# pvachon/tsl-sdr

Measured on AMD Instinct MI355X. Metric: input IQ MSamp/s x channels demodulated, higher is better.
Workload: dtype int16

## Files before the change

tsl-sdr_amd/csrc/mfm_flex.hip:

```cpp
#include <hip/hip_runtime.h>

#include <cstdio>
#include <cstring>
#include <new>
#include <vector>

#include "../../include/multifm_hip.h"
#include "mfm_bch.h"

extern "C" __attribute__((visibility("hidden"))) void mfm_internal_set_error(const char *msg);

namespace {

constexpr uint32_t FX_HIST = 32768;
constexpr uint32_t FX_DEAD = 311;
constexpr uint32_t FX_MATCH_WORDS = 256;
constexpr uint32_t FX_HALO_WORDS = 10;
constexpr uint32_t FX_GATHER_THREADS = 256;

enum : uint32_t { FX_SEARCH = 0, FX_SYNC1 = 1, FX_FRAME = 2 };

struct FxCoding {
    uint16_t seq_a, baud;
    uint8_t levels, skip, fudge, nr_phases;
    uint16_t sync2, symbols;
};
__device__ const FxCoding fx_codings[4] = {
    { 0x78f3, 1600, 2, 9, 0, 1, 40, 2816 },
    { 0x84e7, 3200, 2, 4, 2, 2, 80, 5632 },
    { 0x4f97, 3200, 4, 9, 0, 2, 40, 2816 },
    { 0x215f, 6400, 4, 4, 2, 4, 80, 5632 },
};

struct FxIn {
    const int16_t *x;
    size_t stride;
    const int16_t *hist;
    uint64_t base, end;
};

__device__ __forceinline__ int fx_sample(const FxIn &I, uint32_t c, uint64_t s)
{
    const int16_t *in_block = I.x + (size_t)c * I.stride + (size_t)(s - I.base);
    const int16_t *in_ring = I.hist + (size_t)c * FX_HIST + (size_t)(s & (FX_HIST - 1));
    return *(s >= I.base ? in_block : in_ring);
}


struct __attribute__((packed, aligned(2))) FxPcm8 {
    int16_t v[8];
};

__device__ __forceinline__ uint32_t fx_sign8(const FxIn &I, uint32_t c, int64_t s)
{
    uint32_t b = 0;
    if (s >= (int64_t)I.base && (uint64_t)s + 8 <= I.end) {
        const FxPcm8 p = *reinterpret_cast<const FxPcm8 *>(I.x + (size_t)c * I.stride + (size_t)((uint64_t)s - I.base));
#pragma unroll
        for (int i = 0; i < 8; i++) {
            b |= (uint32_t)(p.v[i] >= 0) << i;
        }
    } else if (s >= 0 && (uint64_t)s + 8 <= I.base) {
        const uint4 q = *reinterpret_cast<const uint4 *>(I.hist + (size_t)c * FX_HIST + (size_t)((uint64_t)s & (FX_HIST - 1)));
        const uint32_t w[4] = { q.x, q.y, q.z, q.w };
#pragma unroll
        for (int i = 0; i < 4; i++) {
            b |= (uint32_t)((w[i] & 0x8000u) == 0) << (2 * i);
            b |= (uint32_t)((w[i] & 0x80000000u) == 0) << (2 * i + 1);
        }
    } else {
        for (int i = 0; i < 8; i++) {
            const int64_t si = s + i;
            if (si >= 0 && (uint64_t)si < I.end) {
                b |= (uint32_t)(fx_sample(I, c, (uint64_t)si) >= 0) << i;
            }
        }
    }
    return b;
}

__global__ __launch_bounds__(256) void fx_match_kernel(const FxIn I, uint32_t *M, uint32_t mstride, uint64_t *SUM, uint32_t sstride,
                                                       uint64_t w0, uint32_t nwords)
{
    __shared__ uint32_t bits[FX_MATCH_WORDS + FX_HALO_WORDS + 2];
    uint8_t *bytes = reinterpret_cast<uint8_t *>(bits);
    const uint32_t c = blockIdx.y, wb = blockIdx.x * FX_MATCH_WORDS, t = threadIdx.x;
    const int64_t s_first = ((int64_t)(w0 + wb) - (int64_t)FX_HALO_WORDS) * 32;
    for (uint32_t g = t; g < 4 * (FX_MATCH_WORDS + FX_HALO_WORDS); g += 256) {
        bytes[g] = (uint8_t)fx_sign8(I, c, s_first + 8 * (int64_t)g);
    }
    if (t == 0) {
        bits[FX_MATCH_WORDS + FX_HALO_WORDS] = 0;
    }
    __syncthreads();
    uint32_t m = 0;
    if (wb + t < nwords) {
        m = 0xffffffffu;
#pragma unroll
        for (uint32_t k = 0; k < 32; k++) {
            const uint32_t off = 32 * FX_HALO_WORDS + 32 * t - 10 * k;
            const uint32_t v = __funnelshift_r(bits[off >> 5], bits[(off >> 5) + 1], off & 31);
            m &= (k & 1) ? v : ~v;
        }
        const uint64_t i0 = (w0 + wb + t) * 32;
        if (i0 + 32 > I.end) {
            m &= (I.end > i0) ? (0xffffffffu >> (32 - (uint32_t)(I.end - i0))) : 0u;
        }
        M[(size_t)c * mstride + wb + t] = m;
    }
    const uint64_t any = __ballot(m != 0);
    if ((t & 63) == 0 && wb + t < nwords) {
        SUM[(size_t)c * sstride + ((wb + t) >> 6)] = any;
    }
}


struct FxState {
    uint64_t p;
    uint64_t j;
    uint32_t mode;
    uint32_t run;
    uint32_t eye;
    uint32_t coding;
    uint32_t a, b, inv_a, fiw_raw, fiw;
    int32_t range, delta;
    uint32_t cycle, frame, pad;
};

struct FxFrameDesc {
    uint64_t first;
    uint32_t coding;
    int32_t range, delta;
    uint32_t pad;
};

struct FxWalk {
    FxIn I;
    const uint32_t *M;
    const uint64_t *SUM;
    uint32_t mstride, sstride, nwords;
    uint64_t w0;
    FxState *st;
    mfm_flex_event *ev;
    mfm_flex_frame_words *fw;
    struct FxFrameDesc *fd;
    uint32_t *counts;
    uint32_t max_ev, max_fw;
    const MfmBchTables *bch;
};

__device__ __forceinline__ int fx_wave_sum(int v)
{
#pragma unroll
    for (int d = 32; d >= 1; d >>= 1) {
        v += __shfl_xor(v, d);
    }
    return v;
}

__device__ __forceinline__ uint32_t fx_checksum(uint32_t w)
{
    w &= 0x1fffffu;
    uint32_t s = 0;
#pragma unroll
    for (int n = 0; n < 6; n++) {
        s += (w >> (4 * n)) & 0xfu;
    }
    return s & 0xfu;
}

__device__ __forceinline__ uint32_t fx_slice4(int v, int delta, int range)
{
    const int s = (int16_t)(v - delta);
    if (s < 0) {
        return (-s > range / 4) ? 0u : 1u;
    }
    return (s > range / 4) ? 2u : 3u;
}

__device__ void fx_emit(const FxWalk &L, uint32_t c, uint32_t &nev, uint32_t type, uint64_t sample, const FxState &S, uint32_t fiw_rc,
                        uint32_t frame_index)
{
    if (nev < L.max_ev && threadIdx.x == 0) {
        mfm_flex_event e;
        e.type = type;
        e.channel = c;
        e.sample = sample;
        e.sync_sample = (type == MFM_FLEX_EV_FRAME) ? S.j : 0;
        e.coding = S.coding;
        e.baud = (S.coding < 4) ? fx_codings[S.coding].baud : 0;
        e.eye = S.eye;
        e.a = S.a;
        e.b = S.b;
        e.inv_a = S.inv_a;
        e.fiw_raw = S.fiw_raw;
        e.fiw = S.fiw;
        e.fiw_rc = fiw_rc;
        e.sample_range = S.range;
        e.sample_delta = S.delta;
        e.cycle = S.cycle;
        e.frame = S.frame;
        e.frame_index = frame_index;
        e.nr_phases = (S.coding < 4) ? fx_codings[S.coding].nr_phases : 0;
        e.reserved = 0;
        L.ev[(size_t)c * L.max_ev + nev] = e;
    }
    nev++;
}

__global__ __launch_bounds__(64) void fx_walk_kernel(const FxWalk L)
{
    const uint32_t c = blockIdx.x, lane = threadIdx.x;
    const FxIn &I = L.I;
    const uint64_t end = I.end;
    const uint32_t *M = L.M + (size_t)c * L.mstride;
    const uint64_t *SUM = L.SUM + (size_t)c * L.sstride;
    const uint32_t nsum = (L.nwords + 63) >> 6;
    __shared__ MfmBchTables bch_s;
    bool have_bch = false;
    FxState S = L.st[c];
    uint32_t nev = 0, nfw = 0;

    for (;;) {
        if (S.mode == FX_SEARCH) {
            bool opened = false;
            while (S.p < end) {
                if (S.run == 0) {
                    const uint32_t i = (uint32_t)((S.p >> 5) - L.w0);
                    const uint32_t head = M[i] & (0xffffffffu << (S.p & 31));
                    if (head != 0) {
                        S.p = (S.p & ~(uint64_t)31) + ((uint32_t)__ffs((int)head) - 1);
                    } else {
                        const uint32_t j = i + 1, sj = j >> 6;
                        uint64_t v = (sj + lane < nsum) ? SUM[sj + lane] : 0ull;
                        if (lane == 0) {
                            v &= ~0ull << (j & 63);
                        }
                        const uint64_t nz = __ballot(v != 0);
                        if (nz == 0) {
                            const uint64_t next = (L.w0 + (((uint64_t)sj + 64) << 6)) << 5;
                            S.p = next < end ? next : end;
                            continue;
                        }
                        const uint32_t fl = (uint32_t)__ffsll((unsigned long long)nz) - 1;
                        const uint32_t lo = (uint32_t)__shfl((int)(uint32_t)v, (int)fl), hi = (uint32_t)__shfl((int)(uint32_t)(v >> 32), (int)fl);
                        const uint64_t fv = (uint64_t)hi << 32 | lo;
                        const uint32_t wi = ((sj + fl) << 6) + ((uint32_t)__ffsll((unsigned long long)fv) - 1);
                        S.p = ((L.w0 + wi) << 5) + ((uint32_t)__ffs((int)M[wi]) - 1);
                    }
                }
                const uint32_t sh = (uint32_t)(S.p & 31);
                const uint32_t inv = ~(M[(S.p >> 5) - L.w0] >> sh);
                uint32_t avail = 32 - sh;
                if (end - S.p < avail) {
                    avail = (uint32_t)(end - S.p);
                }
                uint32_t ones = (uint32_t)__ffs((int)inv) - 1;
                if (inv == 0) {
                    ones = 32;
                }
                if (ones > avail) {
                    ones = avail;
                }
                S.run += ones;
                S.p += ones;
                if (ones < avail) {
                    const uint32_t cnt = S.run & 255u;
                    S.run = 0;
                    if (cnt >= 3) {
                        S.mode = FX_SYNC1;
                        S.j = S.p;
                        S.eye = cnt;
                        opened = true;
                        break;
                    }
                    S.p += 1;
                }
            }
            if (!opened) {
                break;
            }
        }

        if (S.mode == FX_SYNC1) {
            const uint64_t s0 = S.j + (10 - ((S.eye / 2) % 10));
            if (s0 + 790 >= end) {
                break;
            }
            const bool have_fiw = s0 + 1110 < end;
            const int v0 = fx_sample(I, c, s0 + 10 * lane);
            const uint32_t k1 = 64 + lane;
            const bool use1 = k1 < 80 || (have_fiw && k1 < 112);
            const int v1 = use1 ? fx_sample(I, c, s0 + 10 * k1) : 0;
            const uint64_t bal0 = __ballot(v0 >= 0), bal1 = __ballot(use1 && v1 >= 0);
            S.a = __brev((uint32_t)bal0);
// ... 9 lines not shown
            for (uint32_t i = 0; i < 4; i++) {
                if (S.coding == 0xffffffffu && __popc((uint32_t)fx_codings[i].seq_a ^ (S.a >> 16)) < 4) {
                    S.coding = i;
                }
            }
            if (S.coding == 0xffffffffu) {
                fx_emit(L, c, nev, MFM_FLEX_EV_BAD_BAUD, s0 + 790, S, 0, 0);
                S.mode = FX_SEARCH;
                S.run = 0;
                S.p = s0 + 790 + FX_DEAD;
                continue;
            }
            if (!have_fiw) {
                break;
            }
            S.fiw_raw = (uint32_t)(bal1 >> 16);
            const bool in1 = k1 < 112;
            const int sum_hi = fx_wave_sum((v0 > 0 ? v0 : 0) + (in1 && v1 > 0 ? v1 : 0));
            const int sum_lo = fx_wave_sum((v0 <= 0 ? v0 : 0) + (in1 && v1 <= 0 ? v1 : 0));
            const int n_hi = fx_wave_sum((v0 > 0) + (in1 && v1 > 0));
            const int n_lo = fx_wave_sum((v0 <= 0) + (in1 && v1 <= 0));
            const uint64_t f = s0 + 1110;
            uint32_t rc;
            if (n_hi == 0 || n_lo == 0) {
                rc = 3;
            } else {
                const int high = (int16_t)(sum_hi / n_hi), low = (int16_t)(sum_lo / n_lo);
                S.range = (int16_t)(high - low);
                S.delta = (int16_t)(high - S.range / 2);
                uint32_t bad;
                if (!have_bch) {
                    const uint32_t *src = reinterpret_cast<const uint32_t *>(L.bch);
                    uint32_t *dst = reinterpret_cast<uint32_t *>(&bch_s);
                    for (uint32_t i = lane; i < sizeof(MfmBchTables) / 4u; i += 64u) {
                        dst[i] = src[i];
                    }
                    have_bch = true;
                }
                S.fiw = mfm_bch_fix(&bch_s, S.fiw_raw & 0x7fffffffu, &bad);
                if (bad) {
                    rc = 1;
                } else if (fx_checksum(S.fiw) != 0xfu) {
                    rc = 2;
                } else {
                    rc = 0;
                    S.cycle = (S.fiw >> 4) & 0xfu;
                    S.frame = (S.fiw >> 8) & 0x7fu;
                }
            }
            if (rc != 0) {
                fx_emit(L, c, nev, MFM_FLEX_EV_BAD_FIW, f, S, rc, 0);
                S.mode = FX_SEARCH;
                S.run = 0;
                S.p = f + FX_DEAD;
                continue;
            }
            S.mode = FX_FRAME;
            S.j = f;
        }

        if (S.mode == FX_FRAME) {
            const FxCoding cd = fx_codings[S.coding];
            const uint32_t step = cd.skip + 1u;
            const uint64_t first = S.j + step + cd.fudge + (uint64_t)cd.sync2 * step;
            const uint64_t e = first + (uint64_t)(cd.symbols - 1u) * step;
            if (e >= end) {
                break;
            }
            if (nfw < L.max_fw && nev < L.max_ev && lane == 0) {
                L.fd[(size_t)c * L.max_fw + nfw] = FxFrameDesc{ first, S.coding, S.range, S.delta, 0u };
            }
            fx_emit(L, c, nev, MFM_FLEX_EV_FRAME, e, S, 0, nfw);
            nfw++;
            S.mode = FX_SEARCH;
            S.run = 0;
            S.p = e + FX_DEAD;
        }
    }

    if (lane == 0) {
        L.st[c] = S;
        L.counts[2 * c] = nev;
        L.counts[2 * c + 1] = nfw;
    }
}

__global__ __launch_bounds__(FX_GATHER_THREADS) void fx_gather_kernel(const FxWalk L)
{
    __shared__ uint8_t sym[5632];
    const uint32_t c = blockIdx.y, f = blockIdx.x;
    const uint32_t nfw = L.counts[2 * c + 1] < L.max_fw ? L.counts[2 * c + 1] : L.max_fw;
    if (f >= nfw) {
        return;
    }
    const FxFrameDesc d = L.fd[(size_t)c * L.max_fw + f];
    const FxCoding cd = fx_codings[d.coding];
    const uint32_t step = cd.skip + 1u;
    const bool four = cd.levels == 4;
    uint32_t *out = &L.fw[(size_t)c * L.max_fw + f].words[0][0];
#pragma unroll 11
    for (uint32_t k = threadIdx.x; k < cd.symbols; k += FX_GATHER_THREADS) {
        const int v = fx_sample(L.I, c, d.first + (uint64_t)k * step);
        sym[k] = (uint8_t)(four ? fx_slice4(v, d.delta, d.range) : (uint32_t)(v >= 0));
    }
    __syncthreads();
    for (uint32_t item = threadIdx.x; item < 4 * MFM_FLEX_PHASE_WORDS; item += FX_GATHER_THREADS) {
        const uint32_t q = item / MFM_FLEX_PHASE_WORDS, w = item % MFM_FLEX_PHASE_WORDS;
        bool present;
        uint32_t mul = 1, add = 0, sel = 0;
        if (cd.nr_phases == 1) {
            present = q == 0;
        } else if (cd.nr_phases == 2) {
            present = q == 0 || q == 2;
            if (four) {
                sel = q == 0;
            } else {
                mul = 2;
                add = q >> 1;
            }
        } else {
            present = true;
            mul = 2;
            add = q >> 1;
            sel = (q & 1) == 0;
        }
        uint32_t word = 0;
        if (present) {
            const uint32_t n0 = (w >> 3) * 256 + (w & 7);
#pragma unroll
            for (uint32_t jb = 0; jb < 32; jb++) {
                word |= (((uint32_t)sym[(n0 + 8 * jb) * mul + add] >> sel) & 1u) << jb;
            }
        }
        out[item] = word;
    }
}

__global__ __launch_bounds__(256) void fx_hist_kernel(int16_t *hist, const int16_t *x, size_t stride, uint64_t base, uint32_t n)
{
    const uint32_t c = blockIdx.y, k = blockIdx.x * 256 + threadIdx.x;
    const uint32_t cnt = n < FX_HIST ? n : FX_HIST;
    if (k < cnt) {
        const uint32_t off = n - cnt + k;
        hist[(size_t)c * FX_HIST + (size_t)((base + off) & (FX_HIST - 1))] = x[(size_t)c * stride + off];
    }
}

thread_local char g_fx_error[256] = "";

}

#define FX_TRY(expr)                                                                                         \
    do {                                                                                                     \
        hipError_t err_ = (expr);                                                                            \
        if (err_ != hipSuccess) {                                                                            \
            snprintf(g_fx_error, sizeof(g_fx_error), "%s failed: %s", #expr, hipGetErrorString(err_));       \
            mfm_internal_set_error(g_fx_error);                                                              \
            return MFM_E_DEVICE;                                                                             \
        }                                                                                                    \
    } while (0)

struct mfm_flex {
    mfm_flex_config cfg{};
    uint32_t max_ev = 0, max_fw = 0, mstride = 0, sstride = 0;
    int16_t *d_hist = nullptr;
    uint32_t *d_m = nullptr;
    uint64_t *d_sum = nullptr;
    FxState *d_st = nullptr;
    mfm_flex_event *d_ev = nullptr;
    mfm_flex_frame_words *d_fw = nullptr;
    FxFrameDesc *d_fd = nullptr;
    uint32_t *d_counts = nullptr;
    MfmBchTables *d_bch = nullptr;
    uint64_t total = 0;
    hipStream_t last_stream = nullptr;
    bool have_call = false;
};

extern "C" {

#define FX_TRY_C(expr)                                                                                       \
    do {                                                                                                     \
        hipError_t err_c_ = (expr);                                                                          \
        if (err_c_ != hipSuccess) {                                                                          \
            char msg_c_[256];                                                                                \
            snprintf(msg_c_, sizeof(msg_c_), "%s failed: %s", #expr, hipGetErrorString(err_c_));             \
            mfm_internal_set_error(msg_c_);                                                                  \
            mfm_flex_destroy(pf);                                                                            \
            return MFM_E_DEVICE;                                                                             \
        }                                                                                                    \
    } while (0)

int mfm_flex_create(struct mfm_flex **pf, const struct mfm_flex_config *cfg)
{
    if (!pf || !cfg) {
        return MFM_E_INVAL;
    }
    *pf = nullptr;
    if (cfg->abi_version != MFM_ABI_VERSION || 0 == cfg->nr_channels || 0 == cfg->max_in_samples ||
        cfg->max_in_samples > (1u << 26) || cfg->flags != 0) {
        return MFM_E_INVAL;
    }
    MfmBchTables *d_bch = nullptr;
    const int rc = mfm_internal_bch_device_tables(cfg->device, &d_bch);
    if (rc != MFM_OK) {
        return rc;
    }
    mfm_flex *f = new (std::nothrow) mfm_flex();
    if (!f) {
        return MFM_E_NOMEM;
    }
    f->cfg = *cfg;
    f->d_bch = d_bch;
    f->max_ev = cfg->max_events ? cfg->max_events : cfg->max_in_samples / 1024 + 8;
    f->max_fw = cfg->max_in_samples / 28672 + 2;
    if (f->max_fw > f->max_ev) {
        f->max_fw = f->max_ev;
    }
    f->mstride = cfg->max_in_samples / 32 + 4;
    f->sstride = f->mstride / 64 + 2;
    const size_t C = cfg->nr_channels;
    *pf = f;
    FX_TRY_C(hipSetDevice(cfg->device));
    FX_TRY_C(hipMalloc(&f->d_hist, C * FX_HIST * sizeof(int16_t)));
    FX_TRY_C(hipMemset(f->d_hist, 0, C * FX_HIST * sizeof(int16_t)));
    FX_TRY_C(hipMalloc(&f->d_m, C * f->mstride * sizeof(uint32_t)));
    FX_TRY_C(hipMalloc(&f->d_sum, C * f->sstride * sizeof(uint64_t)));
    FX_TRY_C(hipMalloc(&f->d_st, C * sizeof(FxState)));
    {
        std::vector<FxState> st(C);
        memset(st.data(), 0, C * sizeof(FxState));
        for (size_t c = 0; c < C; c++) {
            st[c].mode = FX_SEARCH;
            st[c].p = FX_DEAD - 1;
        }
        FX_TRY_C(hipMemcpy(f->d_st, st.data(), C * sizeof(FxState), hipMemcpyHostToDevice));
    }
    FX_TRY_C(hipMalloc(&f->d_ev, C * f->max_ev * sizeof(mfm_flex_event)));
    FX_TRY_C(hipMalloc(&f->d_fw, C * f->max_fw * sizeof(mfm_flex_frame_words)));
    FX_TRY_C(hipMalloc(&f->d_fd, C * f->max_fw * sizeof(FxFrameDesc)));
    FX_TRY_C(hipMalloc(&f->d_counts, C * 2 * sizeof(uint32_t)));
    FX_TRY_C(hipMemset(f->d_counts, 0, C * 2 * sizeof(uint32_t)));
    FX_TRY_C(hipDeviceSynchronize());
    return MFM_OK;
}

void mfm_flex_destroy(struct mfm_flex **pf)
{
    if (!pf || !*pf) {
        return;
    }
    mfm_flex *f = *pf;
    (void)hipSetDevice(f->cfg.device);
    (void)hipDeviceSynchronize();
    (void)hipFree(f->d_hist);
    (void)hipFree(f->d_m);
    (void)hipFree(f->d_sum);
    (void)hipFree(f->d_st);
    (void)hipFree(f->d_ev);
    (void)hipFree(f->d_fw);
    (void)hipFree(f->d_fd);
    (void)hipFree(f->d_counts);
    delete f;
    *pf = nullptr;
}

int mfm_flex_process_device(struct mfm_flex *f, const int16_t *d_pcm, size_t in_stride, size_t nr_in, void *stream)
{
    if (!f || (!d_pcm && nr_in) || nr_in > f->cfg.max_in_samples || (nr_in && in_stride < nr_in)) {
        return MFM_E_INVAL;
    }
    hipStream_t s = static_cast<hipStream_t>(stream);
    const uint32_t C = f->cfg.nr_channels, n = (uint32_t)nr_in;
    FX_TRY(hipSetDevice(f->cfg.device));
    if (f->have_call && f->last_stream != s) {
        FX_TRY(hipStreamSynchronize(f->last_stream));
    }
    f->last_stream = s;
    f->have_call = true;
    if (0 == n) {
        FX_TRY(hipMemsetAsync(f->d_counts, 0, (size_t)C * 2 * sizeof(uint32_t), s));
        return MFM_OK;
    }
    const FxIn in{ d_pcm, in_stride, f->d_hist, f->total, f->total + n };
    const uint64_t w0 = in.base >> 5;
    const uint32_t nwords = (uint32_t)(((in.end - 1) >> 5) - w0 + 1);
    hipLaunchKernelGGL(fx_match_kernel, dim3((nwords + FX_MATCH_WORDS - 1) / FX_MATCH_WORDS, C), dim3(256), 0, s, in, f->d_m,
                       f->mstride, f->d_sum, f->sstride, w0, nwords);
    FX_TRY(hipGetLastError());
    const FxWalk W{ in, f->d_m, f->d_sum, f->mstride, f->sstride, nwords, w0, f->d_st, f->d_ev, f->d_fw, f->d_fd, f->d_counts, f->max_ev, f->max_fw, f->d_bch };
    hipLaunchKernelGGL(fx_walk_kernel, dim3(C), dim3(64), 0, s, W);
    FX_TRY(hipGetLastError());
    const uint32_t fw_now = n / 28672u + 2u < f->max_fw ? n / 28672u + 2u : f->max_fw;
    hipLaunchKernelGGL(fx_gather_kernel, dim3(fw_now, C), dim3(FX_GATHER_THREADS), 0, s, W);
    FX_TRY(hipGetLastError());
    const uint32_t cnt = n < FX_HIST ? n : FX_HIST;
    hipLaunchKernelGGL(fx_hist_kernel, dim3((cnt + 255) / 256, C), dim3(256), 0, s, f->d_hist, d_pcm, in_stride, in.base, n);
    FX_TRY(hipGetLastError());
    f->total += n;
    return MFM_OK;
}

int mfm_flex_process_host(struct mfm_flex *f, const int16_t *pcm, size_t in_stride, size_t nr_in)
{
    if (!f || (!pcm && nr_in)) {
        return MFM_E_INVAL;
    }
    FX_TRY(hipSetDevice(f->cfg.device));
    const uint32_t C = f->cfg.nr_channels;
    int16_t *d_in = nullptr;
    FX_TRY(hipMalloc(&d_in, (size_t)C * (nr_in ? nr_in : 1) * 2));
    if (nr_in) {
        FX_TRY(hipMemcpy2D(d_in, nr_in * 2, pcm, in_stride * 2, nr_in * 2, C, hipMemcpyHostToDevice));
    }
    const int rc = mfm_flex_process_device(f, d_in, nr_in, nr_in, nullptr);
    (void)hipDeviceSynchronize();
    (void)hipFree(d_in);
    return rc;
}

int mfm_flex_seek(struct mfm_flex *f, uint64_t samples_before)
{
    if (!f) {
        mfm_internal_set_error("mfm_flex_seek: no object");
        return MFM_E_INVAL;
    }
    if (samples_before >= (1ull << 62)) {
        mfm_internal_set_error("mfm_flex_seek: samples_before must stay below 2^62 (the walk forms int64 differences of positions)");
        return MFM_E_INVAL;
    }
    FX_TRY(hipSetDevice(f->cfg.device));
    if (f->have_call) {
        FX_TRY(hipStreamSynchronize(f->last_stream));
    }
    const size_t C = f->cfg.nr_channels;
    std::vector<FxState> st(C);
    memset(st.data(), 0, C * sizeof(FxState));
    for (size_t c = 0; c < C; c++) {
        st[c].mode = FX_SEARCH;
        st[c].p = samples_before + (FX_DEAD - 1);
    }
    FX_TRY(hipMemset(f->d_hist, 0, C * FX_HIST * sizeof(int16_t)));
    FX_TRY(hipMemcpy(f->d_st, st.data(), C * sizeof(FxState), hipMemcpyHostToDevice));
    FX_TRY(hipMemset(f->d_counts, 0, C * 2 * sizeof(uint32_t)));
    FX_TRY(hipDeviceSynchronize());
    f->total = samples_before;
    f->last_stream = nullptr;
    f->have_call = false;
    return MFM_OK;
}

int mfm_flex_fetch_events(struct mfm_flex *f, struct mfm_flex_event *events, size_t max_events, size_t *nr_events,
                          struct mfm_flex_frame_words *frames, size_t max_frames, size_t *nr_frames)
{
    if (!f || !nr_events || !nr_frames || (!events && max_events) || (!frames && max_frames)) {
        return MFM_E_INVAL;
    }
    *nr_events = 0;
    *nr_frames = 0;
    if (!f->have_call) {
        return MFM_OK;
    }
    FX_TRY(hipSetDevice(f->cfg.device));
    FX_TRY(hipStreamSynchronize(f->last_stream));
    const uint32_t C = f->cfg.nr_channels;
    std::vector<uint32_t> cnt((size_t)C * 2);
    FX_TRY(hipMemcpy(cnt.data(), f->d_counts, (size_t)C * 2 * sizeof(uint32_t), hipMemcpyDeviceToHost));
    size_t tot_ev = 0, tot_fw = 0;
    bool overflow = false;
    for (uint32_t c = 0; c < C; c++) {
        overflow |= cnt[2 * c] > f->max_ev || cnt[2 * c + 1] > f->max_fw;
        tot_ev += cnt[2 * c] > f->max_ev ? f->max_ev : cnt[2 * c];
        tot_fw += cnt[2 * c + 1] > f->max_fw ? f->max_fw : cnt[2 * c + 1];
    }
    *nr_events = tot_ev;
    *nr_frames = tot_fw;
    if (tot_ev > max_events || tot_fw > max_frames) {
        return MFM_E_NOMEM;
    }
    size_t pe = 0, pw = 0;
    for (uint32_t c = 0; c < C; c++) {
        const uint32_t ke = cnt[2 * c] > f->max_ev ? f->max_ev : cnt[2 * c];
        const uint32_t kw = cnt[2 * c + 1] > f->max_fw ? f->max_fw : cnt[2 * c + 1];
        if (ke) {
            FX_TRY(hipMemcpy(events + pe, f->d_ev + (size_t)c * f->max_ev, (size_t)ke * sizeof(mfm_flex_event),
                             hipMemcpyDeviceToHost));
        }
        if (kw) {
            FX_TRY(hipMemcpy(frames + pw, f->d_fw + (size_t)c * f->max_fw, (size_t)kw * sizeof(mfm_flex_frame_words),
                             hipMemcpyDeviceToHost));
        }
        for (uint32_t i = 0; i < ke; i++) {
            mfm_flex_event *e = &events[pe + i];
            if (e->type == MFM_FLEX_EV_FRAME) {
                if (e->frame_index < kw) {
                    e->frame_index += (uint32_t)pw;
                } else {
                    overflow = true;
                    e->frame_index = 0xffffffffu;
                }
            }
        }
        pe += ke;
        pw += kw;
    }
    if (overflow) {
        snprintf(g_fx_error, sizeof(g_fx_error), "a channel produced more than max_events=%u events in one call", f->max_ev);
        mfm_internal_set_error(g_fx_error);
        return MFM_E_STATE;
    }
    return MFM_OK;
}

}
```

tsl-sdr_amd/csrc/mfm_resampler.hip:

```cpp
#include <hip/hip_runtime.h>

#include <cstdio>
#include <cstring>
#include <new>
#include <vector>

#include "../../include/multifm_hip.h"

extern "C" __attribute__((visibility("hidden"))) void mfm_internal_set_error(const char *msg);
#include "mfm_numerics.h"
#include "mfm_rs_plan.h"

namespace {

struct RsLaunch {
    const int16_t *tail;
    const int16_t *pcm;
    int16_t *y;
    const int16_t *phase;
    int16_t *tail_out;
    size_t in_stride;
    uint32_t tail_len, nr_in, tail_cap, out_cap, n_out, plen, interp, decim, p0, nchan, invert;
    uint32_t pos_end, new_tail;
    uint32_t *bits;
    uint32_t bits_stride;
};

template <int BITS>
__device__ __forceinline__ bool rs_pred(int32_t y)
{
    const int16_t s = (int16_t)y;
    return BITS == (int)MFM_BITS_NEG ? s < 0 : s > 0;
}

__device__ __forceinline__ int16_t rs_sample(const RsLaunch &L, uint32_t c, uint32_t v)
{
    int16_t s = 0;
    if (v < L.tail_len) {
        s = L.tail[(size_t)c * L.tail_cap + v];
    } else if (v - L.tail_len < L.nr_in) {
        s = L.pcm[(size_t)c * L.in_stride + (v - L.tail_len)];
    }
    return L.invert ? (int16_t)(-s) : s;
}

template <int NP, int BITS>
__global__ __launch_bounds__(RS_NT) void mfm_resample_kernel(const RsLaunch L)
{
    extern __shared__ __attribute__((aligned(16))) uint8_t rs_smem[];
    uint32_t *ph_s = reinterpret_cast<uint32_t *>(rs_smem);
    const uint32_t npairs = L.plen / 2u;
    int16_t *x_s = reinterpret_cast<int16_t *>(rs_smem + (size_t)L.interp * L.plen * 2u);
    const uint32_t c = blockIdx.y, tid = threadIdx.x;
    const uint32_t j0 = blockIdx.x * RS_OPB;
    const uint32_t j1 = (j0 + RS_OPB < L.n_out ? j0 + RS_OPB : L.n_out) - 1u;
    const uint32_t in_lo = ((L.p0 + j0 * L.decim) / L.interp) & ~1u;
    const uint32_t in_hi = (L.p0 + j1 * L.decim) / L.interp + L.plen + 2u + 8u;
    for (uint32_t i = tid; i < L.interp * npairs; i += RS_NT) {
        ph_s[i] = reinterpret_cast<const uint32_t *>(L.phase)[i];
    }
    for (uint32_t v = in_lo + tid; v < in_hi; v += RS_NT) {
        x_s[v - in_lo] = rs_sample(L, c, v);
    }
    __syncthreads();
    const uint32_t *x32 = reinterpret_cast<const uint32_t *>(x_s);

    const uint32_t t_first = L.p0 + (j0 + tid) * L.decim;
    uint32_t pos_abs = t_first / L.interp, ph = t_first - pos_abs * L.interp;
    const uint32_t step_pos = (RS_NT * L.decim) / L.interp, step_ph = (RS_NT * L.decim) % L.interp;
    constexpr bool REGCOEF = NP > 0;
    uint32_t cw[REGCOEF ? NP : 1];
    if (REGCOEF) {
#pragma unroll
        for (uint32_t i = 0; i < (uint32_t)NP; i++) {
            cw[i] = i < npairs ? ph_s[ph * npairs + i] : 0u;
        }
    }
#pragma unroll
    for (uint32_t u = 0; u < RS_OPT; u++) {
        const uint32_t j = j0 + tid + u * RS_NT;
        if (j >= L.n_out) {
            break;
        }
        const uint32_t pos = pos_abs - in_lo;
        const uint32_t *xw = x32 + (pos >> 1);
        const uint32_t sh = (pos & 1u) * 16u;
        int32_t acc = 0;
        uint32_t lo = xw[0];
        if (REGCOEF) {
#pragma unroll
            for (uint32_t i = 0; i < (uint32_t)NP; i++) {
                const uint32_t hi = xw[i + 1];
                const uint32_t pr = __builtin_amdgcn_alignbit(hi, lo, sh);
                asm("v_dot2_i32_i16 %0, %1, %2, %0" : "+v"(acc) : "v"(pr), "v"(cw[i]));
                lo = hi;
            }
        } else {
            const uint32_t *cp = ph_s + ph * npairs;
            for (uint32_t i = 0; i < npairs; i++) {
                const uint32_t hi = xw[i + 1];
                const uint32_t pr = __builtin_amdgcn_alignbit(hi, lo, sh);
                asm("v_dot2_i32_i16 %0, %1, %2, %0" : "+v"(acc) : "v"(pr), "v"(cp[i]));
                lo = hi;
            }
        }
        asm volatile("s_nop 2" : "+v"(acc));
        if (BITS) {
            const unsigned long long m = __ballot(rs_pred<BITS>(mfm_r14_wide(acc)));
            if ((tid & 31u) == 0) {
                L.bits[(size_t)c * L.bits_stride + (j >> 5)] = (uint32_t)(m >> (tid & 32u));
            }
        } else {
            L.y[(size_t)c * L.out_cap + j] = (int16_t)mfm_r14_wide(acc);
        }
        pos_abs += step_pos;
        ph += step_ph;
        if (ph >= L.interp) {
            ph -= L.interp;
            pos_abs += 1u;
        }
    }
}

__global__ void mfm_rs_tail_kernel(const RsLaunch L)
{
    const uint32_t c = blockIdx.x;
    for (uint32_t i = threadIdx.x; i < L.new_tail; i += blockDim.x) {
        int16_t s = 0;
        const uint32_t v = L.pos_end + i;
        if (v < L.tail_len) {
            s = L.tail[(size_t)c * L.tail_cap + v];
        } else if (v - L.tail_len < L.nr_in) {
            s = L.pcm[(size_t)c * L.in_stride + (v - L.tail_len)];
        }
        L.tail_out[(size_t)c * L.tail_cap + i] = s;
    }
}


typedef int rs_v4i __attribute__((ext_vector_type(4)));

struct RsMLaunch {
    RsLaunch b;
    const rs_v4i *gfrag;
    const int32_t *krow;
    uint32_t R;
    uint32_t rp;
    uint32_t plane;
};

struct __attribute__((packed, aligned(2))) RsPcm8 {
    int16_t v[8];
};

template <int KS, int BITS>
__global__ __launch_bounds__(RSM_NT) void mfm_resample_mfma_kernel(const RsMLaunch M)
{
    extern __shared__ __attribute__((aligned(16))) uint8_t rs_smem[];
    const RsLaunch &L = M.b;
    uint8_t *const pl_h = rs_smem, *const pl_l = rs_smem + M.plane;
    const uint32_t c = blockIdx.y, tid = threadIdx.x, lane = tid & 63u, wave = tid >> 6;
    const uint32_t b0 = blockIdx.x * RSM_NB;
    const uint32_t nrows = RSM_NB + (64u * KS + M.rp - 1u) / M.rp;
    const uint32_t v0 = b0 * M.R;

    const uint32_t g8 = (M.R + 7u) / 8u;
    for (uint32_t it = tid; it < nrows * g8; it += RSM_NT) {
        const uint32_t row = it / g8, grp = it - row * g8;
        const uint32_t v = v0 + row * M.R + 8u * grp;
        uint32_t w[4];
        if (v >= L.tail_len && v + 8u <= L.tail_len + L.nr_in) {
            const RsPcm8 p = *reinterpret_cast<const RsPcm8 *>(L.pcm + (size_t)c * L.in_stride + (v - L.tail_len));
#pragma unroll
            for (int i = 0; i < 4; i++) {
                w[i] = mfm_pack16(p.v[2 * i], p.v[2 * i + 1]);
            }
            if (L.invert) {
#pragma unroll
                for (int i = 0; i < 4; i++) {
                    w[i] = mfm_pack16(-(int32_t)p.v[2 * i], -(int32_t)p.v[2 * i + 1]);
                }
            }
        } else {
#pragma unroll
            for (int i = 0; i < 4; i++) {
                w[i] = mfm_pack16(rs_sample(L, c, v + 2u * (uint32_t)i), rs_sample(L, c, v + 2u * (uint32_t)i + 1u));
            }
        }
        uint2 lo, hi;
        lo.x = __builtin_amdgcn_perm(w[1], w[0], 0x06040200u) ^ 0x80808080u;
        lo.y = __builtin_amdgcn_perm(w[3], w[2], 0x06040200u) ^ 0x80808080u;
        hi.x = __builtin_amdgcn_perm(w[1], w[0], 0x07050301u);
        hi.y = __builtin_amdgcn_perm(w[3], w[2], 0x07050301u);
        const uint32_t at = row * M.rp + 8u * grp;
        *reinterpret_cast<uint2 *>(pl_l + at) = lo;
        *reinterpret_cast<uint2 *>(pl_h + at) = hi;
    }
    __syncthreads();

    const uint32_t kg = lane >> 4, n = lane & 15u;
    rs_v4i a_h[KS], a_l[KS];
#pragma unroll
    for (int ks = 0; ks < KS; ks++) {
        a_h[ks] = M.gfrag[(0 * KS + ks) * 64 + lane];
        a_l[ks] = M.gfrag[(1 * KS + ks) * 64 + lane];
    }
    rs_v4i kr;
#pragma unroll
    for (int i = 0; i < 4; i++) {
        kr[i] = M.krow[4u * kg + (uint32_t)i];
    }
    uint32_t nibw[4] = { 0, 0, 0, 0 };
#pragma unroll
    for (uint32_t g = 0; g < 4; g++) {
        const uint32_t blk = wave * 64u + g * 16u + n;
        const uint32_t off = blk * M.rp + 16u * kg;
        rs_v4i hh = { 0, 0, 0, 0 }, md = hh, ll = hh;
#pragma unroll
        for (int ks = 0; ks < KS; ks++) {
            const rs_v4i b_h = *reinterpret_cast<const rs_v4i *>(pl_h + off + 64u * ks);
            const rs_v4i b_l = *reinterpret_cast<const rs_v4i *>(pl_l + off + 64u * ks);
            hh = __builtin_amdgcn_mfma_i32_16x16x64_i8(a_h[ks], b_h, hh, 0, 0, 0);
            md = __builtin_amdgcn_mfma_i32_16x16x64_i8(a_h[ks], b_l, md, 0, 0, 0);
            ll = __builtin_amdgcn_mfma_i32_16x16x64_i8(a_l[ks], b_l, ll, 0, 0, 0);
            md = __builtin_amdgcn_mfma_i32_16x16x64_i8(a_l[ks], b_h, md, 0, 0, 0);
        }
        const uint32_t j = 16u * (b0 + blk) + 4u * kg;
        int32_t y[4];
#pragma unroll
        for (int i = 0; i < 4; i++) {
            const uint32_t acc = (uint32_t)ll[i] + ((uint32_t)md[i] << 8) + ((uint32_t)hh[i] << 16) + (uint32_t)kr[i];
            y[i] = mfm_r14_wide((int32_t)acc);
        }
        if (BITS) {
            uint32_t nib = 0;
#pragma unroll
            for (int i = 0; i < 4; i++) {
                nib |= (rs_pred<BITS>(y[i]) && j + (uint32_t)i < L.n_out ? 1u : 0u) << i;
            }
            nibw[g] = nib << (16u * (n & 1u) + 4u * kg);
            continue;
        }
        int16_t *dst = L.y + (size_t)c * L.out_cap + j;
        if (j + 4u <= L.n_out) {
            uint2 w;
            w.x = mfm_pack16(y[0], y[1]);
            w.y = mfm_pack16(y[2], y[3]);
            *reinterpret_cast<uint2 *>(dst) = w;
        } else {
#pragma unroll
            for (int i = 0; i < 4; i++) {
                if (j + (uint32_t)i < L.n_out) {
                    dst[i] = (int16_t)y[i];
                }
            }
        }
    }
    if (BITS) {
        const bool b5 = (lane & 32u) != 0u, b4 = (lane & 16u) != 0u;
        uint32_t k0 = b5 ? nibw[2] : nibw[0], k1 = b5 ? nibw[3] : nibw[1];
        k0 |= (uint32_t)__shfl_xor((int)(b5 ? nibw[0] : nibw[2]), 32);
        k1 |= (uint32_t)__shfl_xor((int)(b5 ? nibw[1] : nibw[3]), 32);
        uint32_t k = b4 ? k1 : k0;
        k |= (uint32_t)__shfl_xor((int)(b4 ? k0 : k1), 16);
        k |= (uint32_t)__shfl_xor((int)k, 1);
        const uint32_t wi = (b0 >> 1) + 32u * wave + 8u * kg + (n >> 1);
        if ((n & 1u) == 0u && 32u * wi < L.n_out) {
            L.bits[(size_t)c * L.bits_stride + wi] = k;
        }
    }
}

struct DcState {
    int32_t x_n_1, y_n_1, acc;
};

__global__ __launch_bounds__(64) void mfm_dc_block_kernel(int16_t *y, uint32_t out_cap, uint32_t n_out, uint32_t nchan, int32_t p,
                                                          DcState *st)
{
    const uint32_t c = blockIdx.x * blockDim.x + threadIdx.x;
    if (c >= nchan) {
        return;
    }
    const DcState s0 = st[c];
    uint32_t r = (uint32_t)s0.acc - (uint32_t)s0.x_n_1;
    int32_t yp = s0.y_n_1, xl = 0;
    int16_t *yy = y + (size_t)c * out_cap;
    uint32_t i = 0;
    constexpr uint32_t V = 8;
    if (n_out >= 8u * V) {
        typedef uint32_t u32x4 __attribute__((ext_vector_type(4)));
        const u32x4 *src = reinterpret_cast<const u32x4 *>(yy);
        u32x4 *dst = reinterpret_cast<u32x4 *>(yy);
        u32x4 cur[V], nxt[V];
#pragma unroll
        for (uint32_t k = 0; k < V; k++) {
            cur[k] = src[k];
        }
        const int32_t np = -p;
        for (; i + 8u * V <= n_out; i += 8u * V) {
            const u32x4 *pn = src + (i + 16u * V <= n_out ? i / 8u + V : i / 8u);
#pragma unroll
            for (uint32_t k = 0; k < V; k++) {
                nxt[k] = pn[k];
            }
#pragma unroll
            for (uint32_t k = 0; k < V; k++) {
                const u32x4 w = cur[k];
                u32x4 o;
#pragma unroll
                for (int d = 0; d < 4; d++) {
                    uint32_t acc;
                    r += (uint32_t)__mul24(yp, np);
                    asm("v_mad_i32_i16 %0, %1, %2, %3 op_sel:[0,0,0,0]" : "=v"(acc) : "v"(w[d]), "s"(16384), "v"(r));
                    yp = (int32_t)acc >> 14;
                    const uint32_t lo = (uint32_t)yp;
                    r += (uint32_t)__mul24(yp, np);
                    asm("v_mad_i32_i16 %0, %1, %2, %3 op_sel:[1,0,0,0]" : "=v"(acc) : "v"(w[d]), "s"(16384), "v"(r));
                    yp = (int32_t)acc >> 14;
                    o[d] = __builtin_amdgcn_perm((uint32_t)yp, lo, 0x05040100u);
                }
                xl = (int32_t)w[3] >> 16;
                dst[i / 8u + k] = o;
            }
#pragma unroll
            for (uint32_t k = 0; k < V; k++) {
                cur[k] = nxt[k];
            }
        }
    }
    for (; i < n_out; i++) {
        r -= (uint32_t)p * (uint32_t)yp;
        xl = (int32_t)yy[i];
        yp = (int32_t)(((uint32_t)xl << 14) + r) >> 14;
        yy[i] = (int16_t)yp;
    }
    if (n_out) {
        DcState s;
        s.x_n_1 = (int32_t)((uint32_t)xl << 14);
        s.acc = (int32_t)(((uint32_t)xl << 14) + r);
        s.y_n_1 = yp;
        st[c] = s;
    }
}

thread_local char g_rs_error[256] = "";

}

struct mfm_resampler {
    mfm_resampler_config cfg{};
    RsPlan plan;
// ... 172 lines not shown
        const uint32_t row = kk / p.rp, col = kk % p.rp;
        if (col < p.R) {
            const size_t v = (size_t)row * p.R + col;
            const int32_t s = v < nr_x ? x[v] : 0;
            pl_l[kk] = (int8_t)((s & 0xff) ^ 0x80);
            pl_h[kk] = (int8_t)(s >> 8);
        }
    }
    const int8_t *a_h = t.frag.data() + ((size_t)phase * 2u + 0u) * p.ks * 64u * 16u;
    const int8_t *a_l = t.frag.data() + ((size_t)phase * 2u + 1u) * p.ks * 64u * 16u;
    for (uint32_t q = 0; q < 16; q++) {
        uint32_t hh = 0, md = 0, ll = 0;
        for (uint32_t ks = 0; ks < p.ks; ks++) {
            for (uint32_t kgq = 0; kgq < 4; kgq++) {
                const size_t fa = ((size_t)ks * 64u + kgq * 16u + q) * 16u;
                const uint32_t off = 16u * kgq + 64u * ks;
                for (uint32_t j = 0; j < 16; j++) {
                    const int32_t ah = a_h[fa + j], al = a_l[fa + j], bh = pl_h[off + j], bl = pl_l[off + j];
                    hh += (uint32_t)(ah * bh);
                    md += (uint32_t)(ah * bl) + (uint32_t)(al * bh);
                    ll += (uint32_t)(al * bl);
                }
            }
        }
        const uint32_t acc = ll + (md << 8) + (hh << 16) + (uint32_t)t.krow[(size_t)phase * 16u + q];
        y16[q] = (int16_t)mfm_r14_wide((int32_t)acc);
    }
    return MFM_OK;
}

}

template <int BITS>
static int rs_process(mfm_resampler *r, const int16_t *d_pcm, size_t in_stride, size_t nr_in, hipStream_t s, uint32_t *pn_out)
{
    const uint32_t C = r->cfg.nr_channels, I = r->cfg.interpolate, D = r->cfg.decimate;
    const uint32_t total = r->tail + (uint32_t)nr_in;
    uint32_t n_out = 0;
    if (total > r->plen) {
        const uint64_t lim = (uint64_t)(total - r->plen) * I;
        if (lim > r->phase_id) {
            n_out = (uint32_t)((lim - r->phase_id + D - 1) / D);
        }
    }
    const uint64_t t_end = (uint64_t)r->phase_id + (uint64_t)n_out * D;
    const uint32_t pos_end = (uint32_t)(t_end / I);
    const uint32_t new_tail = total - pos_end;
    RsLaunch L{ r->d_x[r->cur], d_pcm, r->d_y, r->d_phase, r->d_x[r->cur ^ 1], in_stride, r->tail, (uint32_t)nr_in, r->tail_cap,
                r->out_cap, n_out, r->plen, I, D, r->phase_id, C, r->cfg.invert, pos_end, new_tail, r->d_bits, r->bits_stride };
    if (n_out && r->use_mfma) {
        RsMLaunch M{ L, r->d_gfrag + (size_t)r->phase_id * 2u * r->m_ks * 64u, r->d_krow + (size_t)r->phase_id * 16u, r->m_R, r->m_rp,
                     r->m_plane };
        const dim3 grid((n_out + 16u * RSM_NB - 1u) / (16u * RSM_NB), C);
        switch (r->m_ks) {
        case 1: hipLaunchKernelGGL((mfm_resample_mfma_kernel<1, BITS>), grid, dim3(RSM_NT), r->m_lds, s, M); break;
        case 2: hipLaunchKernelGGL((mfm_resample_mfma_kernel<2, BITS>), grid, dim3(RSM_NT), r->m_lds, s, M); break;
        case 3: hipLaunchKernelGGL((mfm_resample_mfma_kernel<3, BITS>), grid, dim3(RSM_NT), r->m_lds, s, M); break;
        default: hipLaunchKernelGGL((mfm_resample_mfma_kernel<4, BITS>), grid, dim3(RSM_NT), r->m_lds, s, M); break;
        }
        RS_TRY(hipGetLastError());
    } else if (n_out) {
        const dim3 grid((n_out + RS_OPB - 1) / RS_OPB, C);
        const uint32_t np4 = r->reg_coef ? (r->plen / 2u + 3u) / 4u : 0u;
        switch (np4) {
        case 1: hipLaunchKernelGGL((mfm_resample_kernel<4, BITS>), grid, dim3(RS_NT), r->lds_bytes, s, L); break;
        case 2: hipLaunchKernelGGL((mfm_resample_kernel<8, BITS>), grid, dim3(RS_NT), r->lds_bytes, s, L); break;
        case 3: hipLaunchKernelGGL((mfm_resample_kernel<12, BITS>), grid, dim3(RS_NT), r->lds_bytes, s, L); break;
        case 4: hipLaunchKernelGGL((mfm_resample_kernel<16, BITS>), grid, dim3(RS_NT), r->lds_bytes, s, L); break;
        case 5: hipLaunchKernelGGL((mfm_resample_kernel<20, BITS>), grid, dim3(RS_NT), r->lds_bytes, s, L); break;
        case 6: hipLaunchKernelGGL((mfm_resample_kernel<24, BITS>), grid, dim3(RS_NT), r->lds_bytes, s, L); break;
        case 7: hipLaunchKernelGGL((mfm_resample_kernel<28, BITS>), grid, dim3(RS_NT), r->lds_bytes, s, L); break;
        case 8: hipLaunchKernelGGL((mfm_resample_kernel<32, BITS>), grid, dim3(RS_NT), r->lds_bytes, s, L); break;
        default: hipLaunchKernelGGL((mfm_resample_kernel<0, BITS>), grid, dim3(RS_NT), r->lds_bytes, s, L); break;
        }
        RS_TRY(hipGetLastError());
    }
    if (n_out && !BITS) {
        if (r->cfg.dc_block) {
            hipLaunchKernelGGL(mfm_dc_block_kernel, dim3((C + 63) / 64), dim3(64), 0, s, r->d_y, r->out_cap, n_out, C,
                               r->dc_p, r->d_dc);
            RS_TRY(hipGetLastError());
        }
    }
    if (new_tail) {
        hipLaunchKernelGGL(mfm_rs_tail_kernel, dim3(C), dim3(64), 0, s, L);
        RS_TRY(hipGetLastError());
    }
    r->phase_id = (uint32_t)(t_end % I);
    r->tail = new_tail;
    r->cur ^= 1;
    *pn_out = n_out;
    return MFM_OK;
}

static int rs_bits_prepare(mfm_resampler *r, uint32_t polarity)
{
    if (polarity != MFM_BITS_NEG && polarity != MFM_BITS_POS) {
        snprintf(g_rs_error, sizeof(g_rs_error), "unknown sign-bit polarity %u (MFM_BITS_NEG or MFM_BITS_POS)", polarity);
        mfm_internal_set_error(g_rs_error);
        return MFM_E_INVAL;
    }
    if (r->cfg.dc_block) {
        snprintf(g_rs_error, sizeof(g_rs_error), "the sign-bit output is not available with the DC blocker: it filters the "
                                                 "resampled PCM in memory, which this form does not write");
        mfm_internal_set_error(g_rs_error);
        return MFM_E_INVAL;
    }
    RS_TRY(hipSetDevice(r->cfg.device));
    if (!r->d_bits) {
        r->bits_stride = ((r->out_cap + 31u) / 32u + 7u) & ~7u;
        RS_TRY(hipMalloc(&r->d_bits, (size_t)r->cfg.nr_channels * r->bits_stride * 4));
    }
    return MFM_OK;
}

extern "C" {

int mfm_resampler_process_device(struct mfm_resampler *r, const int16_t *d_pcm, size_t in_stride, size_t nr_in,
                                 void *stream, int16_t **d_out, size_t *out_stride, size_t *nr_out)
{
    if (!r || !d_pcm || !d_out || !out_stride || !nr_out) {
        return MFM_E_INVAL;
    }
    if (nr_in > r->cfg.max_in_samples) {
        return MFM_E_INVAL;
    }
    RS_TRY(hipSetDevice(r->cfg.device));
    uint32_t n_out = 0;
    const int rc = rs_process<0>(r, d_pcm, in_stride, nr_in, static_cast<hipStream_t>(stream), &n_out);
    if (rc != MFM_OK) {
        return rc;
    }
    *d_out = r->d_y;
    *out_stride = r->out_cap;
    *nr_out = n_out;
    return MFM_OK;
}

int mfm_resampler_process_bits_device(struct mfm_resampler *r, const int16_t *d_pcm, size_t in_stride, size_t nr_in,
                                      void *stream, uint32_t polarity, struct mfm_bits_view *view)
{
    if (!r || !d_pcm || !view || nr_in > r->cfg.max_in_samples) {
        return MFM_E_INVAL;
    }
    int rc = rs_bits_prepare(r, polarity);
    if (rc != MFM_OK) {
        return rc;
    }
    uint32_t n_out = 0;
    rc = polarity == MFM_BITS_NEG ? rs_process<(int)MFM_BITS_NEG>(r, d_pcm, in_stride, nr_in, static_cast<hipStream_t>(stream), &n_out)
                                  : rs_process<(int)MFM_BITS_POS>(r, d_pcm, in_stride, nr_in, static_cast<hipStream_t>(stream), &n_out);
    if (rc != MFM_OK) {
        return rc;
    }
    view->d_bits = r->d_bits;
    view->stride_words = r->bits_stride;
    view->nr_bits = n_out;
    view->polarity = polarity;
    view->reserved = 0;
    return MFM_OK;
}

int mfm_resampler_process_host_to_device(struct mfm_resampler *r, const int16_t *pcm, size_t in_stride, size_t nr_in,
                                         void *stream, int16_t **d_out, size_t *out_stride, size_t *nr_out)
{
    if (!r || (!pcm && nr_in) || nr_in > r->cfg.max_in_samples) {
        return MFM_E_INVAL;
// ... 103 lines not shown
```

Baseline: 36.17 million.

## Fuse flex history refresh, walk and gather kernels; fold resampler tail carry

The history ring update moves into the match kernel, which writes a double-buffered copy so there is no read-after-write hazard, and the separate hist kernel is removed. The per-frame gather is merged into the walk kernel, which now launches 256 threads per channel and gathers frames serially after the 64-lane walk. The resampler tail carry is done by the last block of the resample kernel instead of its own launch. Together these cut kernel launches per call. In exchange, gather parallelism drops from one block per frame to one block per channel, and the walk kernel now uses more threads that sit idle during the walk.

```diff
diff --git a/tsl-sdr_amd/csrc/mfm_flex.hip b/tsl-sdr_amd/csrc/mfm_flex.hip
--- a/tsl-sdr_amd/csrc/mfm_flex.hip
+++ b/tsl-sdr_amd/csrc/mfm_flex.hip
@@ -79,8 +79,51 @@
     return b;
 }
 
+__device__ __forceinline__ void fx_ring_refresh(const FxIn &I, int16_t *hist_new, uint32_t c, uint64_t r0, uint32_t t)
+{
+    const uint32_t n = (uint32_t)(I.end - I.base);
+    const int16_t *x = I.x + (size_t)c * I.stride;
+    int16_t *hn = hist_new + (size_t)c * FX_HIST;
+    const uint64_t keep = I.end > FX_HIST ? I.end - FX_HIST : 0;
+    const uint64_t r1 = r0 + 32u * FX_MATCH_WORDS;
+    uint64_t lo = keep > I.base ? keep : I.base, hi = I.end;
+    lo = lo > r0 ? lo : r0;
+    hi = hi < r1 ? hi : r1;
+    for (uint64_t g = (lo & ~(uint64_t)7) + 8u * t; g < hi; g += 8u * 256u) {
+        if (g >= lo && g + 8 <= hi) {
+            const FxPcm8 p = *reinterpret_cast<const FxPcm8 *>(x + (size_t)(g - I.base));
+            uint4 q;
+            q.x = (uint16_t)p.v[0] | (uint32_t)(uint16_t)p.v[1] << 16;
+            q.y = (uint16_t)p.v[2] | (uint32_t)(uint16_t)p.v[3] << 16;
+            q.z = (uint16_t)p.v[4] | (uint32_t)(uint16_t)p.v[5] << 16;
+            q.w = (uint16_t)p.v[6] | (uint32_t)(uint16_t)p.v[7] << 16;
+            *reinterpret_cast<uint4 *>(hn + (size_t)(g & (FX_HIST - 1))) = q;
+        } else {
+            for (uint64_t si = g > lo ? g : lo; si < g + 8 && si < hi; si++) {
+                hn[(size_t)(si & (FX_HIST - 1))] = x[(size_t)(si - I.base)];
+            }
+        }
+    }
+    if (n < FX_HIST) {
+        const int16_t *ho = I.hist + (size_t)c * FX_HIST;
+        const uint32_t old = FX_HIST - n;
+        for (uint32_t gi = blockIdx.x * 256u + t; gi < FX_HIST / 8u; gi += gridDim.x * 256u) {
+            const uint32_t off0 = (8u * gi - (uint32_t)I.end) & (FX_HIST - 1);
+            if (off0 + 7u < old) {
+                *reinterpret_cast<uint4 *>(hn + 8u * gi) = *reinterpret_cast<const uint4 *>(ho + 8u * gi);
+            } else {
+                for (uint32_t i = 0; i < 8u; i++) {
+                    if (((off0 + i) & (FX_HIST - 1)) < old) {
+                        hn[8u * gi + i] = ho[8u * gi + i];
+                    }
+                }
+            }
+        }
+    }
+}
+
 __global__ __launch_bounds__(256) void fx_match_kernel(const FxIn I, uint32_t *M, uint32_t mstride, uint64_t *SUM, uint32_t sstride,
-                                                       uint64_t w0, uint32_t nwords)
+                                                       uint64_t w0, uint32_t nwords, int16_t *hist_new)
 {
     __shared__ uint32_t bits[FX_MATCH_WORDS + FX_HALO_WORDS + 2];
     uint8_t *bytes = reinterpret_cast<uint8_t *>(bits);
@@ -92,6 +135,7 @@
     if (t == 0) {
         bits[FX_MATCH_WORDS + FX_HALO_WORDS] = 0;
     }
+    fx_ring_refresh(I, hist_new, c, (w0 + wb) * 32, t);
     __syncthreads();
     uint32_t m = 0;
     if (wb + t < nwords) {
@@ -208,9 +252,71 @@
     nev++;
 }
 
-__global__ __launch_bounds__(64) void fx_walk_kernel(const FxWalk L)
-{
-    const uint32_t c = blockIdx.x, lane = threadIdx.x;
+__device__ void fx_walk(const FxWalk &L, uint32_t c, uint32_t lane, uint32_t *nfw_out);
+
+__device__ __forceinline__ void fx_gather_frame(const FxWalk &L, uint32_t c, uint32_t f, uint8_t *sym)
+{
+    const FxFrameDesc d = L.fd[(size_t)c * L.max_fw + f];
+    const FxCoding cd = fx_codings[d.coding];
+    const uint32_t step = cd.skip + 1u;
+    const bool four = cd.levels == 4;
+    uint32_t *out = &L.fw[(size_t)c * L.max_fw + f].words[0][0];
+#pragma unroll 11
+    for (uint32_t k = threadIdx.x; k < cd.symbols; k += FX_GATHER_THREADS) {
+        const int v = fx_sample(L.I, c, d.first + (uint64_t)k * step);
+        sym[k] = (uint8_t)(four ? fx_slice4(v, d.delta, d.range) : (uint32_t)(v >= 0));
+    }
+    __syncthreads();
+    for (uint32_t item = threadIdx.x; item < 4 * MFM_FLEX_PHASE_WORDS; item += FX_GATHER_THREADS) {
+        const uint32_t q = item / MFM_FLEX_PHASE_WORDS, w = item % MFM_FLEX_PHASE_WORDS;
+        bool present;
+        uint32_t mul = 1, add = 0, sel = 0;
+        if (cd.nr_phases == 1) {
+            present = q == 0;
+        } else if (cd.nr_phases == 2) {
+            present = q == 0 || q == 2;
+            if (four) {
+                sel = q == 0;
+            } else {
+                mul = 2;
+                add = q >> 1;
+            }
+        } else {
+            present = true;
+            mul = 2;
+            add = q >> 1;
+            sel = (q & 1) == 0;
+        }
+        uint32_t word = 0;
+        if (present) {
+            const uint32_t n0 = (w >> 3) * 256 + (w & 7);
+#pragma unroll
+            for (uint32_t jb = 0; jb < 32; jb++) {
+                word |= (((uint32_t)sym[(n0 + 8 * jb) * mul + add] >> sel) & 1u) << jb;
+            }
+        }
+        out[item] = word;
+    }
+    __syncthreads();
+}
+
+__global__ __launch_bounds__(FX_GATHER_THREADS) void fx_walk_kernel(const FxWalk L)
+{
+    __shared__ uint8_t sym[5632];
+    __shared__ uint32_t nfw_s;
+    const uint32_t c = blockIdx.x;
+    if (threadIdx.x < 64u) {
+        fx_walk(L, c, threadIdx.x, &nfw_s);
+    }
+    __syncthreads();
+    const uint32_t nfw = nfw_s < L.max_fw ? nfw_s : L.max_fw;
+    for (uint32_t f = 0; f < nfw; f++) {
+        fx_gather_frame(L, c, f, sym);
+    }
+}
+
+__device__ void fx_walk(const FxWalk &L, uint32_t c, uint32_t lane, uint32_t *nfw_out)
+{
     const FxIn &I = L.I;
     const uint64_t end = I.end;
     const uint32_t *M = L.M + (size_t)c * L.mstride;
@@ -386,67 +492,7 @@
         L.st[c] = S;
         L.counts[2 * c] = nev;
         L.counts[2 * c + 1] = nfw;
-    }
-}
-
-__global__ __launch_bounds__(FX_GATHER_THREADS) void fx_gather_kernel(const FxWalk L)
-{
-    __shared__ uint8_t sym[5632];
-    const uint32_t c = blockIdx.y, f = blockIdx.x;
-    const uint32_t nfw = L.counts[2 * c + 1] < L.max_fw ? L.counts[2 * c + 1] : L.max_fw;
-    if (f >= nfw) {
-        return;
-    }
-    const FxFrameDesc d = L.fd[(size_t)c * L.max_fw + f];
-    const FxCoding cd = fx_codings[d.coding];
-    const uint32_t step = cd.skip + 1u;
-    const bool four = cd.levels == 4;
-    uint32_t *out = &L.fw[(size_t)c * L.max_fw + f].words[0][0];
-#pragma unroll 11
-    for (uint32_t k = threadIdx.x; k < cd.symbols; k += FX_GATHER_THREADS) {
-        const int v = fx_sample(L.I, c, d.first + (uint64_t)k * step);
-        sym[k] = (uint8_t)(four ? fx_slice4(v, d.delta, d.range) : (uint32_t)(v >= 0));
-    }
-    __syncthreads();
-    for (uint32_t item = threadIdx.x; item < 4 * MFM_FLEX_PHASE_WORDS; item += FX_GATHER_THREADS) {
-        const uint32_t q = item / MFM_FLEX_PHASE_WORDS, w = item % MFM_FLEX_PHASE_WORDS;
-        bool present;
-        uint32_t mul = 1, add = 0, sel = 0;
-        if (cd.nr_phases == 1) {
-            present = q == 0;
-        } else if (cd.nr_phases == 2) {
-            present = q == 0 || q == 2;
-            if (four) {
-                sel = q == 0;
-            } else {
-                mul = 2;
-                add = q >> 1;
-            }
-        } else {
-            present = true;
-            mul = 2;
-            add = q >> 1;
-            sel = (q & 1) == 0;
-        }
-        uint32_t word = 0;
-        if (present) {
-            const uint32_t n0 = (w >> 3) * 256 + (w & 7);
-#pragma unroll
-            for (uint32_t jb = 0; jb < 32; jb++) {
-                word |= (((uint32_t)sym[(n0 + 8 * jb) * mul + add] >> sel) & 1u) << jb;
-            }
-        }
-        out[item] = word;
-    }
-}
-
-__global__ __launch_bounds__(256) void fx_hist_kernel(int16_t *hist, const int16_t *x, size_t stride, uint64_t base, uint32_t n)
-{
-    const uint32_t c = blockIdx.y, k = blockIdx.x * 256 + threadIdx.x;
-    const uint32_t cnt = n < FX_HIST ? n : FX_HIST;
-    if (k < cnt) {
-        const uint32_t off = n - cnt + k;
-        hist[(size_t)c * FX_HIST + (size_t)((base + off) & (FX_HIST - 1))] = x[(size_t)c * stride + off];
+        *nfw_out = nfw;
     }
 }
 
@@ -467,7 +513,8 @@
 struct mfm_flex {
     mfm_flex_config cfg{};
     uint32_t max_ev = 0, max_fw = 0, mstride = 0, sstride = 0;
-    int16_t *d_hist = nullptr;
+    int16_t *d_hist[2] = { nullptr, nullptr };
+    int cur = 0;
     uint32_t *d_m = nullptr;
     uint64_t *d_sum = nullptr;
     FxState *d_st = nullptr;
@@ -526,8 +573,10 @@
     const size_t C = cfg->nr_channels;
     *pf = f;
     FX_TRY_C(hipSetDevice(cfg->device));
-    FX_TRY_C(hipMalloc(&f->d_hist, C * FX_HIST * sizeof(int16_t)));
-    FX_TRY_C(hipMemset(f->d_hist, 0, C * FX_HIST * sizeof(int16_t)));
+    for (int i = 0; i < 2; i++) {
+        FX_TRY_C(hipMalloc(&f->d_hist[i], C * FX_HIST * sizeof(int16_t)));
+        FX_TRY_C(hipMemset(f->d_hist[i], 0, C * FX_HIST * sizeof(int16_t)));
+    }
     FX_TRY_C(hipMalloc(&f->d_m, C * f->mstride * sizeof(uint32_t)));
     FX_TRY_C(hipMalloc(&f->d_sum, C * f->sstride * sizeof(uint64_t)));
     FX_TRY_C(hipMalloc(&f->d_st, C * sizeof(FxState)));
@@ -557,7 +606,8 @@
     mfm_flex *f = *pf;
     (void)hipSetDevice(f->cfg.device);
     (void)hipDeviceSynchronize();
-    (void)hipFree(f->d_hist);
+    (void)hipFree(f->d_hist[0]);
+    (void)hipFree(f->d_hist[1]);
     (void)hipFree(f->d_m);
     (void)hipFree(f->d_sum);
     (void)hipFree(f->d_st);
@@ -586,21 +636,16 @@
         FX_TRY(hipMemsetAsync(f->d_counts, 0, (size_t)C * 2 * sizeof(uint32_t), s));
         return MFM_OK;
     }
-    const FxIn in{ d_pcm, in_stride, f->d_hist, f->total, f->total + n };
+    const FxIn in{ d_pcm, in_stride, f->d_hist[f->cur], f->total, f->total + n };
     const uint64_t w0 = in.base >> 5;
     const uint32_t nwords = (uint32_t)(((in.end - 1) >> 5) - w0 + 1);
     hipLaunchKernelGGL(fx_match_kernel, dim3((nwords + FX_MATCH_WORDS - 1) / FX_MATCH_WORDS, C), dim3(256), 0, s, in, f->d_m,
-                       f->mstride, f->d_sum, f->sstride, w0, nwords);
+                       f->mstride, f->d_sum, f->sstride, w0, nwords, f->d_hist[f->cur ^ 1]);
     FX_TRY(hipGetLastError());
     const FxWalk W{ in, f->d_m, f->d_sum, f->mstride, f->sstride, nwords, w0, f->d_st, f->d_ev, f->d_fw, f->d_fd, f->d_counts, f->max_ev, f->max_fw, f->d_bch };
-    hipLaunchKernelGGL(fx_walk_kernel, dim3(C), dim3(64), 0, s, W);
+    hipLaunchKernelGGL(fx_walk_kernel, dim3(C), dim3(FX_GATHER_THREADS), 0, s, W);
     FX_TRY(hipGetLastError());
-    const uint32_t fw_now = n / 28672u + 2u < f->max_fw ? n / 28672u + 2u : f->max_fw;
-    hipLaunchKernelGGL(fx_gather_kernel, dim3(fw_now, C), dim3(FX_GATHER_THREADS), 0, s, W);
-    FX_TRY(hipGetLastError());
-    const uint32_t cnt = n < FX_HIST ? n : FX_HIST;
-    hipLaunchKernelGGL(fx_hist_kernel, dim3((cnt + 255) / 256, C), dim3(256), 0, s, f->d_hist, d_pcm, in_stride, in.base, n);
-    FX_TRY(hipGetLastError());
+    f->cur ^= 1;
     f->total += n;
     return MFM_OK;
 }
@@ -644,7 +689,7 @@
         st[c].mode = FX_SEARCH;
         st[c].p = samples_before + (FX_DEAD - 1);
     }
-    FX_TRY(hipMemset(f->d_hist, 0, C * FX_HIST * sizeof(int16_t)));
+    FX_TRY(hipMemset(f->d_hist[f->cur], 0, C * FX_HIST * sizeof(int16_t)));
     FX_TRY(hipMemcpy(f->d_st, st.data(), C * sizeof(FxState), hipMemcpyHostToDevice));
     FX_TRY(hipMemset(f->d_counts, 0, C * 2 * sizeof(uint32_t)));
     FX_TRY(hipDeviceSynchronize());
diff --git a/tsl-sdr_amd/csrc/mfm_resampler.hip b/tsl-sdr_amd/csrc/mfm_resampler.hip
--- a/tsl-sdr_amd/csrc/mfm_resampler.hip
+++ b/tsl-sdr_amd/csrc/mfm_resampler.hip
@@ -44,6 +44,25 @@
     return L.invert ? (int16_t)(-s) : s;
 }
 
+__device__ __forceinline__ void rs_carry(const RsLaunch &L, uint32_t c, uint32_t tid, uint32_t nthreads)
+{
+    for (uint32_t i = tid; i < L.new_tail; i += nthreads) {
+        int16_t s = 0;
+        const uint32_t v = L.pos_end + i;
+        if (v < L.tail_len) {
+            s = L.tail[(size_t)c * L.tail_cap + v];
+        } else if (v - L.tail_len < L.nr_in) {
+            s = L.pcm[(size_t)c * L.in_stride + (v - L.tail_len)];
+        }
+        L.tail_out[(size_t)c * L.tail_cap + i] = s;
+    }
+}
+
+__global__ void mfm_rs_tail_kernel(const RsLaunch L)
+{
+    rs_carry(L, blockIdx.x, threadIdx.x, blockDim.x);
+}
+
 template <int NP, int BITS>
 __global__ __launch_bounds__(RS_NT) void mfm_resample_kernel(const RsLaunch L)
 {
@@ -120,20 +139,8 @@
             pos_abs += 1u;
         }
     }
-}
-
-__global__ void mfm_rs_tail_kernel(const RsLaunch L)
-{
-    const uint32_t c = blockIdx.x;
-    for (uint32_t i = threadIdx.x; i < L.new_tail; i += blockDim.x) {
-        int16_t s = 0;
-        const uint32_t v = L.pos_end + i;
-        if (v < L.tail_len) {
-            s = L.tail[(size_t)c * L.tail_cap + v];
-        } else if (v - L.tail_len < L.nr_in) {
-            s = L.pcm[(size_t)c * L.in_stride + (v - L.tail_len)];
-        }
-        L.tail_out[(size_t)c * L.tail_cap + i] = s;
+    if (blockIdx.x + 1u == gridDim.x) {
+        rs_carry(L, c, tid, RS_NT);
     }
 }
 
@@ -268,6 +275,9 @@
         if ((n & 1u) == 0u && 32u * wi < L.n_out) {
             L.bits[(size_t)c * L.bits_stride + wi] = k;
         }
+    }
+    if (blockIdx.x + 1u == gridDim.x) {
+        rs_carry(L, c, tid, RSM_NT);
     }
 }
 
@@ -606,7 +616,7 @@
             RS_TRY(hipGetLastError());
         }
     }
-    if (new_tail) {
+    if (new_tail && !n_out) {
         hipLaunchKernelGGL(mfm_rs_tail_kernel, dim3(C), dim3(64), 0, s, L);
         RS_TRY(hipGetLastError());
     }
```

Result: no change. 36.16 million (-0.0%).
